# tejank10/AlphaGo.jl

Measured on AMD Instinct MI355X. Metric: self-play positions/sec (9x9, tower=10, 400 readouts), higher is better.
Workload: dtype f32

## Files before the change

alphago.jl_amd/csrc/agz_nn.h:

```cpp
#pragma once
#include <algorithm>
#include <cstdint>
#include <functional>
#include <memory>
#include <vector>

#include "agz_common.h"

namespace agz {

constexpr int kC = 256;
constexpr int kCinStem = 17;
constexpr int kCinStemPad = 32;

struct ConvHost {
  int k = 3, cin = 0, cout = 0;
  std::vector<float> w, b, beta, gamma, mean, var;
  float eps = 1e-5f;
};
struct DenseHost {
  int in = 0, out = 0;
  std::vector<float> w, b;
};

// ... 57 lines not shown
  uint64_t param_version() const { return param_version_; }

  double flops_per_eval() const;
  double conv_flops_per_launch(int B) const { return 2.0 * B * P_ * 9.0 * kC * kC; }

 private:
  void pack();
  void stem(TowerForm form, const float* d_x32, const int* d_count, int bcap);
  void direct_tower(const int* d_count, int bcap);
  void f16_tower(const int* d_count, int bcap);
  void wino_tower(TowerForm form, const int* d_count, int bcap);
  void persistent_tower(const int* d_count, int bcap);
  struct LayerIO { const float *vin, *res; float *y, *vout; };
  LayerIO layer_io(int l, bool dense) const;
  void wino_layer(TowerForm form, int l, const LayerIO& io, const int* d_count, int bcap, hipStream_t st, int part = 0,
                  int parts = 1);
  template <class Layer> void run_chains(int chains, const Layer& layer);
  template <class Launch> void timed(int layers, const Launch& launch);

  int N_, P_, A_, tower_;
  hipStream_t stream_;
  ConvHost stem_, vconv_, pconv_;
  std::vector<ConvHost> tconv_;
  DenseHost vfc1_, vfc2_, pfc_;
  struct FluxSlot { int layer, kind; size_t off, n; };
  std::vector<FluxSlot> slots_;
  size_t flux_n_ = 0;
  DevBuf<float> d_flux_;
  bool derived_dirty_ = true;
  mutable bool host_stale_ = false;
  uint64_t param_version_ = 0;
  void upload_slot(const FluxSlot& s);
  void upload_host_all();
  const float* host_slot(const FluxSlot& s) const;

  DevBuf<float> d_wstem_, d_wtower_;
  DevBuf<float> d_scale_, d_shift_;
  DevBuf<float> d_head_;
  const float *d_vfc1w_ = nullptr, *d_vfc1b_ = nullptr, *d_vfc2w_ = nullptr, *d_vfc2b_ = nullptr, *d_pfcw_ = nullptr,
              *d_pfcb_ = nullptr;
  int bcap_ = 0;
  DevBuf<float> d_a_, d_b_, d_t_, d_vh_, d_ph_;
  int winograd_ = 1;
  DevBuf<float> d_uwino5_;
  bool packed5_ = false;
  DevBuf<float> d_uwino4_;
  bool packed4_ = false;
  static constexpr int kMaxTowerStreams = 4;
  int tower_streams_ = 2;
  hipStream_t streamx_[kMaxTowerStreams - 1] = {nullptr, nullptr, nullptr};
  hipEvent_t ev_fork_ = nullptr, ev_join_[kMaxTowerStreams - 1] = {nullptr, nullptr, nullptr};
  DevBuf<float> d_uwino_s_, d_scale_s_;
  bool packed_split_ = false;
  DevBuf<float> d_uwino_, d_vimg_, d_vimg2_;
  DevBuf<float> d_ustem_, d_ustem_s_;
  int precision_ = 0;
  bool packed16_ = false;
// ... 53 lines not shown
inline void wino_block_range(int blocks, int part, int parts, bool pairs, int& tb0, int& tb1) {
  AGZ_REQUIRE(parts >= 1 && part >= 0 && part < parts, AGZ_BAD_ARGUMENT, "tile-block range %d of %d", part, parts);
  int per = (blocks + parts - 1) / parts;
  if (pairs) per = (per + 1) & ~1;
  tb0 = std::min(blocks, part * per);
  tb1 = part + 1 == parts ? blocks : std::min(blocks, tb0 + per);
}
inline void wino_check_32bit(long blocks, int rows, int bcap, int N) {
  AGZ_REQUIRE((blocks + 1) * rows < (1L << 31) && (long)bcap * N * N * kC * 4 < (1L << 32), AGZ_BAD_ARGUMENT,
              "batch of %d positions at %dx%d: tile index / activation byte offset exceeds 32 bits", bcap, N, N);
}
void launch_wino_in(const float* x, float* vimg, const int* d_count, int bcap, int N, bool split, hipStream_t s,
                    int ns = kWinoStages, bool fixup = false);
void launch_wino_gemm(const float* vimg, const float* uimg, const float* scale, const float* shift, const float* res,
                      float* y, float* vnext, const int* d_count, int bcap, int N, int relu, bool split, hipStream_t s,
                      int ns = kWinoStages, int part = 0, int parts = 1);
bool wino_fusable(int N);
struct WinoTowerLayer {
  const float *v, *u, *scale, *shift, *res;
  float *y, *vnext;
  int mode, relu;
};
size_t wino_tower_sched_ints(int layers, int bcap, int N);
bool wino_tower_supported(hipStream_t s);
void launch_wino_tower(const void* d_layers, int layers, int* d_sched, const int* d_count, int bcap, int N, bool split, hipStream_t s);
constexpr int kWinoTowerErrWord = 8;
void wino_pack_weights_split(const ConvHost& c, float* out, int ns = kWinoStages);
float wino_split_descale();

void wino5_pack_weights(const ConvHost& c, float* out);
void launch_wino5_pack(const float* d_w, long wstride, int layers, float* d_out, hipStream_t s);
size_t wino5_weight_floats();
void launch_wino5_gemm(const float* vimg, const float* uimg, const float* scale, const float* shift, const float* res,
                       float* y, float* vnext, const int* d_count, int bcap, int N, int relu, hipStream_t s, int part = 0,
                       int parts = 1);

// ... 29 lines not shown
```

alphago.jl_amd/csrc/agz_nn.hip:

```cpp
#include "agz_nn.h"

#include <cmath>
#include <algorithm>
#include <cstring>

#include "../../include/agz_draws.h"

namespace agz {

typedef float f32x16 __attribute__((ext_vector_type(16)));


constexpr int BM = 128, BN = 128, BK = 32;
constexpr int LDS_STRIDE = BK + 4;

template <int CIN, bool TAPSPLIT = false>
__global__ __launch_bounds__(256, 2) void k_conv3x3_mfma(
    const float* __restrict__ x, const float* __restrict__ wt, const float* __restrict__ scale,
    const float* __restrict__ shift, const float* __restrict__ res, float* __restrict__ y,
    const int* __restrict__ d_count, int N, int relu, long ystride = 0) {
  constexpr int NCHUNK = 9 * CIN / BK;
  constexpr int CPT = CIN / BK;
  const int c_begin = TAPSPLIT ? (int)blockIdx.y * CPT : 0, c_end = TAPSPLIT ? c_begin + CPT : NCHUNK;
  if (TAPSPLIT) y += (long)blockIdx.y * ystride;
// ... 143 lines not shown
  const int lane = threadIdx.x & 63, wave = threadIdx.x >> 6;
#pragma unroll
  for (int o = 32; o > 0; o >>= 1) {
    const float t = __shfl_xor(v, o, 64);
    v = is_max ? fmaxf(v, t) : v + t;
  }
  __syncthreads();
  if (lane == 0) red[wave] = v;
  __syncthreads();
  float r = red[0];
#pragma unroll
  for (int w = 1; w < 4; ++w) r = is_max ? fmaxf(r, red[w]) : r + red[w];
  return r;
}

__global__ __launch_bounds__(256) void k_head_fc(
    const float* __restrict__ vh, const float* __restrict__ ph, const float* __restrict__ w1,
    const float* __restrict__ b1, const float* __restrict__ w2, const float* __restrict__ b2,
    const float* __restrict__ wp, const float* __restrict__ bp, float* __restrict__ pi,
    float* __restrict__ v, const int* __restrict__ d_count, int P, int A) {
  extern __shared__ __attribute__((aligned(16))) float sm[];
  float* vin = sm;
  float* pin = sm + P;
  float* logit = pin + 2 * P;
  float* red = logit + A;
  const int b = blockIdx.x;
  if (b >= *d_count) return;
  const int tid = threadIdx.x;
  for (int i = tid; i < P; i += 256) {
    vin[i] = vh[(long)b * P + i];
    pin[i] = ph[((long)b * P + i) * 2 + 0];
    pin[P + i] = ph[((long)b * P + i) * 2 + 1];
  }
  __syncthreads();
  float lmax = -INFINITY;
  for (int o = tid; o < A; o += 256) {
    float z = bp[o];
    for (int i = 0; i < 2 * P; ++i) z += wp[o + (long)A * i] * pin[i];
    logit[o] = z;
    lmax = fmaxf(lmax, z);
  }
  const float mx = block_reduce(lmax, true, red);
  float lsum = 0.f;
  for (int o = tid; o < A; o += 256) {
    const float e = expf(logit[o] - mx);
    logit[o] = e;
    lsum += e;
  }
  const float sum = block_reduce(lsum, false, red);
  for (int o = tid; o < A; o += 256) pi[(long)b * A + o] = logit[o] / sum;
  float h = b1[tid];
  for (int i = 0; i < P; ++i) h += w1[tid + 256 * i] * vin[i];
  h = fmaxf(h, 0.f);
  const float s = block_reduce(h * w2[tid], false, red);
  if (tid == 0) v[b] = tanhf(s + b2[0]);
}


__global__ __launch_bounds__(128) void k_feats_from_deltas(
    const int8_t* __restrict__ boards, const int8_t* __restrict__ deltas, const int32_t* __restrict__ ndeltas,
    const int8_t* __restrict__ to_play, int B, int N, float* __restrict__ x32, float* __restrict__ whcn) {
  const int b = blockIdx.x;
  if (b >= B) return;
  const int P = N * N;
  const int nd = ndeltas[b];
  const int tp = to_play[b];
  for (int p = threadIdx.x; p < P; p += blockDim.x) {
    int cur = boards[(long)b * P + p];
    float f[32];
#pragma unroll
// ... 447 lines not shown

void Net::reserve(int bcap) {
  if (precision_ == 1 && tower_ > 0 && d_ha_.n < ((size_t)std::max(bcap, bcap_) * P_ + 256) * kC) {
    const size_t n = ((size_t)std::max(bcap, bcap_) * P_ + 256) * kC;
    d_ha_.alloc(n);
    d_hb_.alloc(n);
    d_ht_.alloc(n);
  }
  if (bcap <= bcap_) return;
  const size_t rows = (size_t)bcap * P_;
  d_a_.alloc(rows * kC);
  d_b_.alloc(rows * kC);
  d_t_.alloc(rows * kC);
  d_vh_.alloc(rows);
  d_ph_.alloc(rows * 2);
  if (tower_ > 0) {
    const size_t vf = std::max(wino_v_floats(bcap, (N_ + 2) / 3), wino4_applies(N_) ? wino4_v_floats(bcap, N_) : (size_t)0);
    d_vimg_.alloc(vf);
    d_vimg2_.alloc(vf);
  }
  bcap_ = bcap;
}

static inline int conv_grid(int bcap, int P) { return ceil_div((long)bcap * P, BM) * (kC / BN); }
int conv3x3_direct_blocks(int bcap, int N) { return conv_grid(bcap, N * N); }

void launch_conv3x3_direct(const float* x, const float* wt, const float* scale, const float* shift, const float* res,
                           float* y, const int* d_count, int bcap, int N, int relu, int cin_pad, hipStream_t s) {
  const int grid = conv_grid(bcap, N * N);
  if (cin_pad == kCinStemPad)
// ... 143 lines not shown
    timed(1, [&] {
      launch_conv16_dma(d_ht_.p, d_wi16_.p + iper * l2, sc + (size_t)l2 * kC, sh + (size_t)l2 * kC,
                        first ? (const void*)a : (const void*)cur, first ? 1 : 0, last ? (void*)d_b_.p : (void*)nxt,
                        last ? 1 : 0, d_count, bcap, N_, 1, stream_);
    });
    std::swap(cur, nxt);
  }
}

Net::LayerIO Net::layer_io(int l, bool dense) const {
  if (l % 2 == 0) return {d_vimg_.p, nullptr, dense ? d_t_.p : nullptr, d_vimg2_.p};
  const bool odd = (l / 2) % 2;
  return {d_vimg2_.p, odd ? d_b_.p : d_a_.p, odd ? d_a_.p : d_b_.p, l + 1 == 2 * tower_ ? nullptr : d_vimg_.p};
}

void Net::wino_layer(TowerForm form, int l, const LayerIO& io, const int* d_count, int bcap, hipStream_t st, int part, int parts) {
  const float* sc = d_scale_.p + (size_t)(l + 1) * kC;
  const float* sh = d_shift_.p + (size_t)(l + 1) * kC;
  if (form == TowerForm::Wino4) {
    launch_wino4_gemm(io.vin, d_uwino4_.p + wino4_weight_floats() * l, sc, sh, io.res, io.y, io.vout, d_count, bcap, N_, 1, st,
                      part, parts, io.y && !io.res && wino4_paired(N_));
    if (io.vout && !wino4_whole_boards(N_)) launch_wino4_in(io.y, io.vout, d_count, bcap, N_, st, true, part, parts);
  } else if (form == TowerForm::Wino5) {
    launch_wino5_gemm(io.vin, d_uwino5_.p + wino5_weight_floats() * l, sc, sh, io.res, io.y, io.vout, d_count, bcap, N_, 1, st,
                      part, parts);
  } else {
    const bool split = precision_ == 2;
    const float* u = (split ? d_uwino_s_.p : d_uwino_.p) + wino_weight_floats() * l;
    launch_wino_gemm(io.vin, u, split ? d_scale_s_.p + (size_t)l * kC : sc, sh, io.res, io.y, io.vout, d_count, bcap, N_, 1, split,
                     st, kWinoStages, part, parts);
    if (io.vout && !wino_fusable(N_)) launch_wino_in(io.y, io.vout, d_count, bcap, N_, split, st, kWinoStages, true);
  }
}

void Net::wino_tower(TowerForm form, const int* d_count, int bcap) {
  const bool f44 = form == TowerForm::Wino4;
  const bool dense = f44 ? !wino4_whole_boards(N_) : !wino_fusable(N_);
  const int T = f44 ? (N_ + 3) / 4 : (N_ + 2) / 3;
  const int chains = dense && !f44 ? 1 : chain_count(tower_streams_, (long)bcap * T * T, f44 ? 64 : 63);
  run_chains(chains, [&](int l, int part, hipStream_t st) {
    wino_layer(form, l, layer_io(l, dense), d_count, bcap, st, part, chains);
  });
}

void Net::persistent_tower(const int* d_count, int bcap) {
  const bool split = precision_ == 2;
  const float* usrc = split ? d_uwino_s_.p : d_uwino_.p;
  const float* sc = split ? d_scale_s_.p : d_scale_.p + kC;
  const float* sh = d_shift_.p + kC;
  const int nl = 2 * tower_;
  std::vector<WinoTowerLayer> tab(nl);
  for (int l = 0; l < nl; ++l) {
    const LayerIO io = layer_io(l, false);
    tab[l] = {io.vin, usrc + wino_weight_floats() * l, sc + (size_t)l * kC, sh + (size_t)l * kC, io.res, io.y, io.vout,
              (io.y ? 1 : 0) | (io.vout ? 2 : 0), 1};
  }
  const size_t tbytes = sizeof(WinoTowerLayer) * tab.size();
  if (tower_layers_host_.size() != tbytes || std::memcmp(tower_layers_host_.data(), tab.data(), tbytes) != 0) {
    AGZ_HIP(hipStreamSynchronize(stream_));
    tower_layers_host_.assign((const char*)tab.data(), (const char*)tab.data() + tbytes);
    d_tower_layers_.ensure(tbytes);
    AGZ_HIP(hipMemcpy(d_tower_layers_.p, tower_layers_host_.data(), tbytes, hipMemcpyHostToDevice));
  }
  d_tower_sched_.ensure(wino_tower_sched_ints(nl, bcap, N_));
  if (!tower_err_) {
    AGZ_HIP(hipHostMalloc((void**)&tower_err_, sizeof(int32_t), hipHostMallocDefault));
    *tower_err_ = 0;
  }
  timed(nl, [&] { launch_wino_tower(d_tower_layers_.p, nl, d_tower_sched_.p, d_count, bcap, N_, split, stream_); });
  (void)hipMemcpyAsync(tower_err_, d_tower_sched_.p + kWinoTowerErrWord, sizeof(int32_t), hipMemcpyDeviceToHost, stream_);
// ... 3 lines not shown
  check_async_error();
  TowerForm form = tower_form();
  if (form == TowerForm::Wino4) wino4_validate(bcap, N_);
  pack();
  reserve(bcap);
  if (prof_on_ && prof_fwd_ < kProfMax)
    (void)hipMemcpyAsync(&prof_counts_[prof_fwd_], d_count, sizeof(int32_t), hipMemcpyDeviceToHost, stream_);
  stem(form, d_x32, d_count, bcap);
  if (form == TowerForm::Wino3Persistent && !wino_tower_supported(stream_)) form = TowerForm::Wino3;
  switch (form) {
    case TowerForm::Direct: direct_tower(d_count, bcap); break;
    case TowerForm::F16: f16_tower(d_count, bcap); break;
    case TowerForm::Wino3Persistent: persistent_tower(d_count, bcap); break;
    default: wino_tower(form, d_count, bcap); break;
  }
  const float* x = form == TowerForm::F16 || tower_ % 2 ? d_b_.p : d_a_.p;
  const int hgrid = std::min(ceil_div((long)bcap * P_, 4), 256 * 16);
  hipLaunchKernelGGL(k_head_conv, dim3(hgrid), dim3(256), 0, stream_, x, d_head_.p, d_vh_.p, d_ph_.p, d_count, P_);
  const size_t smem = sizeof(float) * (size_t)(3 * P_ + A_ + 4);
  hipLaunchKernelGGL(k_head_fc, dim3(bcap), dim3(256), smem, stream_, (const float*)d_vh_.p,
                     (const float*)d_ph_.p, d_vfc1w_, d_vfc1b_, d_vfc2w_, d_vfc2b_, d_pfcw_,
                     d_pfcb_, d_pi, d_v, d_count, P_, A_);
  if (prof_on_ && prof_fwd_ < kProfMax) prof_fwd_++;
  AGZ_HIP(hipGetLastError());
}

__global__ __launch_bounds__(256) void k_mfma_f32_sustained(int iters, float* out) {
  typedef float f32x16 __attribute__((ext_vector_type(16)));
  f32x16 acc[8];
#pragma unroll
  for (int i = 0; i < 8; ++i)
#pragma unroll
    for (int e = 0; e < 16; ++e) acc[i][e] = 0.f;
  const float a = 1.f + threadIdx.x * 1e-6f, b = 0.5f;
  for (int it = 0; it < iters; ++it) {
#pragma unroll
    for (int i = 0; i < 8; ++i) acc[i] = __builtin_amdgcn_mfma_f32_32x32x2f32(a, b, acc[i], 0, 0, 0);
// ... 143 lines not shown
```

alphago.jl_amd/csrc/agz_wino.hip:

```cpp
#include "agz_nn.h"
#include "agz_glds.h"

#include <algorithm>
#include <cmath>
#include <cstdio>
#include <cstdlib>
#include <cstring>
#include <type_traits>

namespace agz {

typedef float f32x16 __attribute__((ext_vector_type(16)));

constexpr int WT = 64;
constexpr int WC = 64;
constexpr int WK = 4;
constexpr int WNS = kC / WK;
static_assert(WNS == kWinoStages && kCinStemPad == kWinoStemStages * WK, "stage counts of agz_nn.h");
constexpr int WXI = 25;
constexpr int WPL = 13;
constexpr int A_STAGE = WPL * WT * 8;
constexpr int B_STAGE = WPL * WC * 8;
constexpr int STAGE = A_STAGE + B_STAGE;

__host__ __device__ __forceinline__ int wino_v_off(int xi, int row, int h) {
  return (xi >> 1) * (WT * 8) + (xi & 1) * (WT * 4) + row * 4 + 2 * ((h + (row >> 4)) & 1);
}

typedef _Float16 h8 __attribute__((ext_vector_type(8)));
typedef _Float16 h4 __attribute__((ext_vector_type(4)));
constexpr float kSplitV = 8.f, kSplitU = 1024.f;
__host__ __device__ __forceinline__ void split_half(float x, _Float16& hi, _Float16& lo) {
  hi = (_Float16)x;
  lo = (_Float16)(x - (float)hi);
// ... 11 lines not shown
  const int lo = (ti > 0 ? T : 0) + (tj > 0 ? 1 : 0), hi = (ti < T - 1 ? T : 0) + (tj < T - 1 ? 1 : 0);
  return row - lo >= 0 && row + hi < WT;
}


__device__ __forceinline__ void bt5(float x0, float x1, float x2, float x3, float x4, float* r) {
  r[3] = x3 - x1;
  r[0] = __builtin_fmaf(2.f, x0 - x2, r[3]);
  r[4] = __builtin_fmaf(-2.f, r[3], x4 - x2);
  r[1] = __builtin_fmaf(2.f, x1, x2 - x3);
  r[2] = __builtin_fmaf(-2.f, x1, __builtin_fmaf(3.f, x2, -x3));
}

template <int TPB, bool NT, bool SPLIT = false, int NS = WNS, bool FIXUP = false>
__global__ __launch_bounds__(256) void k_wino_in(const float* __restrict__ x, float* __restrict__ vimg,
                                                  const int* __restrict__ d_count, int N, int T) {
  static_assert(TPB == 32, "the copy-out below moves 32-row chunks");
  constexpr int LPT = 256 / TPB;
  constexpr int SP = LPT / 2;
  constexpr int CH = TPB * 4;
  constexpr int IMG = 26 * CH + 8;
  __shared__ __attribute__((aligned(16))) float img[SP * IMG];
  const int P = N * N, TT = T * T;
  const int RPB = wino_rows_per_block(T);
  const long Mt = (long)(*d_count) * TT;
  constexpr int PARTS = WT / TPB;
  const int tb = blockIdx.x / PARTS, part = blockIdx.x % PARTS;
  if ((long)tb * RPB + part * TPB >= Mt) return;
  const int hs = threadIdx.x % LPT, h = hs & 1, sl = hs >> 1;
  const int tl = threadIdx.x / LPT;
  const int row = part * TPB + tl;
// ... 11 lines not shown
      const bool ok = live && pi >= 0 && pi < N && pj >= 0 && pj < N;
      off[u * 5 + v] = ok ? (b * P + pi + N * pj) * (NS * WK) : -1;
    }
  float* mine = img + sl * IMG + tl * 4 + (SPLIT ? 0 : 2 * ((h + (row >> 4)) & 1));
  if (SPLIT) { mine[25 * CH + h] = 0.f; mine[25 * CH + 2 + h] = 0.f; }
  else *reinterpret_cast<float2*>(mine + 25 * CH) = make_float2(0.f, 0.f);
  float* gdst = vimg + (long)tb * NS * A_STAGE + part * CH;
  const int cq = threadIdx.x / TPB, cl = threadIdx.x % TPB;
  bool copy_row = true;
  if (FIXUP) {
    const int crow = part * TPB + cl;
    const long ctile = (long)tb * RPB + crow;
    const int ct = (int)(ctile % TT);
    copy_row = !(crow < RPB && ctile < Mt && wino_tile_fused(T, crow, ct / T, ct % T));
  }
  for (int sg = 0; sg < NS / SP; ++sg) {
    const int st = sg * SP + sl;
    float2 d[25];
#pragma unroll
    for (int q = 0; q < 25; ++q)
      d[q] = off[q] >= 0 ? *reinterpret_cast<const float2*>(x + off[q] + st * WK + 2 * h) : make_float2(0.f, 0.f);
    float tx[25], ty[25];
#pragma unroll
    for (int v = 0; v < 5; ++v) {
      float r[5];
      bt5(d[0 * 5 + v].x, d[1 * 5 + v].x, d[2 * 5 + v].x, d[3 * 5 + v].x, d[4 * 5 + v].x, r);
#pragma unroll
      for (int i = 0; i < 5; ++i) tx[i * 5 + v] = r[i];
      bt5(d[0 * 5 + v].y, d[1 * 5 + v].y, d[2 * 5 + v].y, d[3 * 5 + v].y, d[4 * 5 + v].y, r);
#pragma unroll
      for (int i = 0; i < 5; ++i) ty[i * 5 + v] = r[i];
    }
    if (sg) __syncthreads();
#pragma unroll
    for (int i = 0; i < 5; ++i) {
      float rx[5], ry[5];
// ... 9 lines not shown
          *reinterpret_cast<h2*>(mine + (i * 5 + j) * CH + h) = (h2){xh, yh};
          *reinterpret_cast<h2*>(mine + (i * 5 + j) * CH + 2 + h) = (h2){xl, yl};
        } else {
          *reinterpret_cast<float2*>(mine + (i * 5 + j) * CH) = make_float2(rx[j], ry[j]);
        }
      }
    }
    __syncthreads();
#pragma unroll
    for (int r = 0; r < 13; ++r) {
      const int c = r * 8 + cq, s4 = c / 26, xi = c % 26;
      typedef float f32x4 __attribute__((ext_vector_type(4)));
      const f32x4 v = *reinterpret_cast<const f32x4*>(img + s4 * IMG + xi * CH + cl * 4);
      f32x4* gp = reinterpret_cast<f32x4*>(gdst + (long)(sg * SP + s4) * A_STAGE + (xi >> 1) * (WT * 8) + (xi & 1) * (WT * 4) + cl * 4);
      if (FIXUP && !copy_row) continue;
      if (NT) __builtin_nontemporal_store(v, gp);
      else *gp = v;
    }
  }
}

constexpr int IMG_FLOATS = WT * 9 * WC;

template <bool SPLIT, int NS, bool COH>
__device__ __forceinline__ void wino_wg(
    float* __restrict__ lds, int* __restrict__ ptab, const float* __restrict__ vimg, const float* __restrict__ uimg,
    const float* __restrict__ scale, const float* __restrict__ shift, const float* __restrict__ res, float* __restrict__ y,
    float* __restrict__ vnext, const long Mt, const int N, const int T, const int relu, const int tb, const int cb, const int MODE,
    const int tid) {
  const int P = N * N, TT = T * T;
  const int RPB = wino_rows_per_block(T);
  const int lane = tid & 63;
  const int wave = __builtin_amdgcn_readfirstlane(tid >> 6);
  const int wm = wave & 1, wn = wave >> 1;
  const int l31 = lane & 31, hi = lane >> 5;
  const float* asrc = vimg + (long)tb * NS * A_STAGE;
  const float* bsrc = uimg + (long)cb * NS * B_STAGE;
  const unsigned lds0 = (unsigned)(size_t)(__attribute__((address_space(3))) float*)&lds[0];

  auto dma = [&](int st, int buf, int j) {
    const int c = 13 * wave + j;
    if (j == 12 && (wave & 1)) return;
    const float* g = wave < 2 ? asrc + (long)st * A_STAGE + c * 256 : bsrc + (long)st * B_STAGE + (c - 26) * 256;
    if constexpr (COH) glds16s_l2(g, (unsigned)lane * 16u, lds0 + (unsigned)(buf * STAGE + c * 256) * 4u);
// ... 110 lines not shown
      if (t < WXI) load(L, t, ra[t % RING], rb[t % RING]);
      else if (next) load(Ln, t - WXI, ra[t % RING], rb[t % RING]);
      constexpr int D0 = SPLIT ? 0 : 6;
      if (more && k >= D0 && k < D0 + PW) {
        __builtin_amdgcn_sched_barrier(0);
        dma(st + 2, dbuf, k - D0);
        __builtin_amdgcn_sched_barrier(0);
      }
      if (first) mma0(k, ra[k % RING], rb[k % RING]);
      else mma(k, ra[k % RING], rb[k % RING]);
    }
    buf = nbuf;
  };
  static_assert(NS >= 4, "stage 0 is peeled off the loop");
  stage(0, std::true_type{}, std::true_type{}, std::true_type{});
  for (int st = 1; st < NS - 2; ++st) stage(st, std::true_type{}, std::true_type{}, std::false_type{});
  stage(NS - 2, std::false_type{}, std::true_type{}, std::false_type{});
  stage(NS - 1, std::false_type{}, std::false_type{}, std::false_type{});

  static_assert(WXI == 25, "the pad below lists the accumulators of transform columns 3 and 4");
  asm volatile("s_nop 15\n\ts_nop 15"
               : "+v"(acc[3]), "+v"(acc[4]), "+v"(acc[8]), "+v"(acc[9]), "+v"(acc[13]), "+v"(acc[14]), "+v"(acc[18]),
                 "+v"(acc[19]), "+v"(acc[23]), "+v"(acc[24]));

  __syncthreads();
  float* img = lds;
  static_assert(IMG_FLOATS + WC <= 3 * STAGE, "tile image (+ the block of zeros phase 2 reads for off-board points) exceeds the stage buffers");
  if (tid < WC) img[IMG_FLOATS + tid] = 0.f;
  const bool pass1b = (MODE & 1) != 0;
  if (res) {
    static_assert(WT * 9 / 4 == 4 * 36, "36 residual pieces per wave");
#pragma unroll
    for (int n = 0; n < 36; ++n) rdma(n);
  }
  {
    const int col = wn * 32 + l31;
    const float sc = scale[cb * WC + col], sh = shift[cb * WC + col];
    const float relu_lo = relu ? 0.f : -3.0e38f;
    f32x16 o[9];
    {
      f32x16 tmp[3][5];
#pragma unroll
      for (int jj = 0; jj < 5; ++jj) {
        const int j = (jj + 3) % 5;
// ... 32 lines not shown
            rr[ee][k] = decltype(with_res)::value ? *((lds_f*)(size_t)pa[ee][k >> 2] + (k & 3) * (WT * WC)) : 0.f;
        }
#pragma unroll
        for (int ee = 0; ee < 4; ++ee)
#pragma unroll
          for (int k = 0; k < 9; ++k) {
            float v = o[k][e0 + ee] * sc + sh + rr[ee][k];
            v = fmaxf(v, relu_lo);
            *((lds_f*)(size_t)pa[ee][k >> 2] + (k & 3) * (WT * WC)) = v;
          }
      }
    };
    if (res) rows(std::true_type{});
    else rows(std::false_type{});
  }
  __syncthreads();
  typedef float f32x4 __attribute__((ext_vector_type(4)));
  if (pass1b) {
    constexpr int PER = WT * 9 * (WC / 4) / 256;
    const int cg4 = 4 * ((tid ^ (tid >> 4)) & 15);
    f32x4* ip0 = reinterpret_cast<f32x4*>(img) + tid;
    const int* pt0 = ptab + (tid >> 4);
    int offs[PER];
#pragma unroll
    for (int i = 0; i < PER; ++i) offs[i] = pt0[16 * i];
#pragma unroll
    for (int i0 = 0; i0 < PER; i0 += 12) {
      f32x4 v[12];
#pragma unroll
      for (int j = 0; j < 12; ++j) v[j] = ip0[256 * (i0 + j)];
#pragma unroll
      for (int j = 0; j < 12; ++j)
        if ((MODE & 1) && offs[i0 + j] >= 0) *reinterpret_cast<f32x4*>(y + offs[i0 + j] + cg4) = v[j];
// ... 83 lines not shown
          v4 = __builtin_bit_cast(f32x4, pk);
        } else {
          v4 = (f32x4){p0[0], p0[1], p1[0], p1[1]};
        }
        f32x4* gp = reinterpret_cast<f32x4*>(g + (xi >> 1) * (WT * 8) + (xi & 1) * (WT * 4));
        if (emit) __builtin_nontemporal_store(v4, gp);
      }
    }
  }
}

template <int MODE, bool SPLIT = false, int NS = WNS>
__global__ __launch_bounds__(256, 1) void k_wino_gemm4(
    const float* __restrict__ vimg, const float* __restrict__ uimg, const float* __restrict__ scale,
    const float* __restrict__ shift, const float* __restrict__ res, float* __restrict__ y,
    float* __restrict__ vnext, const int* __restrict__ d_count, int N, int T, int relu, int tb0, int tb1) {
  __shared__ __attribute__((aligned(256))) float lds[3 * STAGE];
  __shared__ int ptab[WT * 9];
  const long Mt = (long)(*d_count) * (T * T);
  const int bid = blockIdx.x;
  const int xcd = bid & 7, jb = bid >> 3;
  const int cb = jb & 3;
  const int tb = tb0 + xcd + 8 * (jb >> 2);
  if (tb >= tb1 || (long)tb * wino_rows_per_block(T) >= Mt) return;
  wino_wg<SPLIT, NS, false>(lds, ptab, vimg, uimg, scale, shift, res, y, vnext, Mt, N, T, relu, tb, cb, MODE, (int)threadIdx.x);
}

typedef WinoTowerLayer TowerLayer;
static_assert(kWinoTowerErrWord == 8, "");
constexpr int kTowerErr = kWinoTowerErrWord, kTowerDone = 64;
constexpr int kTowerSpinLimit = 1 << 22;

template <bool SPLIT>
__global__ __launch_bounds__(256, 1) void k_wino_tower(const TowerLayer* __restrict__ layers, int nl, int* __restrict__ sched,
                                                       int blocks_cap, const int* __restrict__ d_count, int N, int T, int order) {
  __shared__ __attribute__((aligned(256))) float lds[3 * STAGE];
  __shared__ int ptab[WT * 9];
  __shared__ int s_bc;
  const int tid = threadIdx.x;
  unsigned xcc;
// ... 31 lines not shown
      int spins = 0;
      while (__hip_atomic_load(flag, __ATOMIC_RELAXED, __HIP_MEMORY_SCOPE_AGENT) < 4) {
        __builtin_amdgcn_s_sleep(8);
        if (++spins > kTowerSpinLimit || ((spins & 1023) == 0 && __hip_atomic_load(&sched[kTowerErr], __ATOMIC_RELAXED, __HIP_MEMORY_SCOPE_AGENT))) {
          atomicOr(&sched[kTowerErr], 2);
          s_bc = 1;
          break;
        }
      }
    }
    __syncthreads();
    if (s_bc) return;
    const TowerLayer L = layers[l];
    int t = tid;
    asm volatile("" : "+v"(t));
    wino_wg<SPLIT, WNS, true>(lds, ptab, L.v, L.u, L.scale, L.shift, L.res, L.y, L.vnext, Mt, N, T, L.relu, tb, cb, L.mode, t);
    asm volatile("s_waitcnt vmcnt(0)" ::: "memory");
    __syncthreads();
    if (tid == 0) {
      int* flag = done + (size_t)l * blocks_cap + tb;
      if (__hip_atomic_fetch_add(flag, 1, __ATOMIC_RELAXED, __HIP_MEMORY_SCOPE_AGENT) != 3) {
        int spins = 0;
        while (__hip_atomic_load(flag, __ATOMIC_RELAXED, __HIP_MEMORY_SCOPE_AGENT) < 4 && ++spins < kTowerSpinLimit) __builtin_amdgcn_s_sleep(2);
      }
    }
  }
}

__global__ void k_xcd_census(int* out) {
  __shared__ float hog[150 * 1024 / 4];
  unsigned xcc;
// ... 67 lines not shown

size_t wino_weight_floats(int ns) { return (size_t)(kC / WC) * ns * B_STAGE; }
long wino_blocks(int bcap, int T) {
  const long rpb = wino_rows_per_block(T);
  return ((long)bcap * T * T + rpb - 1) / rpb;
}
size_t wino_v_floats(int bcap, int T) { return (size_t)wino_blocks(bcap, T) * WNS * A_STAGE; }
bool wino_fusable(int N) { return wino_whole_boards((N + 2) / 3); }

void launch_wino_in(const float* x, float* vimg, const int* d_count, int bcap, int N, bool split, hipStream_t s, int ns,
                    bool fixup) {
  const int T = (N + 2) / 3;
  const int blocks = (int)wino_blocks(bcap, T);
  AGZ_REQUIRE(!fixup || (ns == kWinoStages && !wino_whole_boards(T)), AGZ_BAD_ARGUMENT, "fix-up transform: dense tile blocks, tower layers");
#define WIN_LAUNCH(SPLIT_, NS_, FIXUP_) \
  hipLaunchKernelGGL((k_wino_in<32, true, SPLIT_, NS_, FIXUP_>), dim3(2 * blocks), dim3(256), 0, s, x, vimg, d_count, N, T)
  constexpr int S = kWinoStemStages;
  switch ((fixup ? 4 : ns == S ? 2 : 0) | (split ? 1 : 0)) {
    case 5: WIN_LAUNCH(true, WNS, true); break;
    case 4: WIN_LAUNCH(false, WNS, true); break;
    case 3: WIN_LAUNCH(true, S, false); break;
    case 2: WIN_LAUNCH(false, S, false); break;
    case 1: WIN_LAUNCH(true, WNS, false); break;
    default: WIN_LAUNCH(false, WNS, false); break;
  }
#undef WIN_LAUNCH
}

void launch_wino_gemm(const float* vimg, const float* uimg, const float* scale, const float* shift, const float* res,
                      float* y, float* vnext, const int* d_count, int bcap, int N, int relu, bool split, hipStream_t s, int ns, int part,
                      int parts) {
  const int T = (N + 2) / 3;
  const int all_blocks = (int)wino_blocks(bcap, T);
  int tb0, tb1;
  wino_block_range(all_blocks, part, parts, false, tb0, tb1);
  AGZ_REQUIRE(parts == 1 || wino_whole_boards(T), AGZ_BAD_ARGUMENT, "F(3x3,3x3): %d layer chains need whole-board tile blocks", parts);
  if (tb1 <= tb0) return;
  const int blocks = tb1 - tb0;
  const int per_xcd = 4 * ((blocks + 7) / 8);
  const dim3 grid(8 * per_xcd), block(256);
  wino_check_32bit(all_blocks, WT, bcap, N);
  const bool stem = ns == kWinoStemStages;
  const int mode = vnext ? (y || stem ? 3 : 2) : 1;
#define WG_LAUNCH(MODE_, SPLIT_, NS_)                                                                                     \
  hipLaunchKernelGGL((k_wino_gemm4<MODE_, SPLIT_, NS_>), grid, block, 0, s, vimg, uimg, scale, shift, res, y, vnext, d_count, \
                     N, T, relu, tb0, tb1)
  constexpr int S = kWinoStemStages;
  switch (mode | (split ? 4 : 0) | (stem ? 8 : 0)) {
    case 15: WG_LAUNCH(3, true, S); break;
    case 13: WG_LAUNCH(1, true, S); break;
    case 11: WG_LAUNCH(3, false, S); break;
    case 9: WG_LAUNCH(1, false, S); break;
    case 7: WG_LAUNCH(3, true, WNS); break;
    case 6: WG_LAUNCH(2, true, WNS); break;
    case 5: WG_LAUNCH(1, true, WNS); break;
    case 3: WG_LAUNCH(3, false, WNS); break;
    case 2: WG_LAUNCH(2, false, WNS); break;
    default: WG_LAUNCH(1, false, WNS); break;
  }
#undef WG_LAUNCH
}
// ... 44 lines not shown
```

Before: 447.1.

## Fuse head 1x1 convs into last Winograd layer epilogue and trim stem stages

The last tower layer's Winograd GEMM epilogue now computes per-channel-block partial dot products for the value and policy 1x1 head convolutions, instead of writing the full activation. A new head FC kernel sums the four partials and applies BN/ReLU, which removes the separate head-conv launch and the full-activation write and read. The stem Winograd transform and GEMM also now process only the stages that cover the real 17 input channels rather than the padded 32. This adds a partial-sum buffer and epilogue complexity, and the fused path only applies when boards split into whole tile blocks.

```diff
diff --git a/alphago.jl_amd/csrc/agz_nn.h b/alphago.jl_amd/csrc/agz_nn.h
--- a/alphago.jl_amd/csrc/agz_nn.h
+++ b/alphago.jl_amd/csrc/agz_nn.h
@@ -95,7 +95,10 @@
   struct LayerIO { const float *vin, *res; float *y, *vout; };
   LayerIO layer_io(int l, bool dense) const;
   void wino_layer(TowerForm form, int l, const LayerIO& io, const int* d_count, int bcap, hipStream_t st, int part = 0,
-                  int parts = 1);
+                  int parts = 1, bool heads = false);
+  bool heads_fused(TowerForm form) const {
+    return (form == TowerForm::Wino3 || form == TowerForm::Wino3Persistent) && tower_ >= 1 && wino_fusable(N_);
+  }
   template <class Layer> void run_chains(int chains, const Layer& layer);
   template <class Launch> void timed(int layers, const Launch& launch);
 
@@ -122,6 +125,7 @@
               *d_pfcb_ = nullptr;
   int bcap_ = 0;
   DevBuf<float> d_a_, d_b_, d_t_, d_vh_, d_ph_;
+  DevBuf<float> d_hpart_;
   int winograd_ = 1;
   DevBuf<float> d_uwino5_;
   bool packed5_ = false;
@@ -205,12 +209,16 @@
                     int ns = kWinoStages, bool fixup = false);
 void launch_wino_gemm(const float* vimg, const float* uimg, const float* scale, const float* shift, const float* res,
                       float* y, float* vnext, const int* d_count, int bcap, int N, int relu, bool split, hipStream_t s,
-                      int ns = kWinoStages, int part = 0, int parts = 1);
+                      int ns = kWinoStages, int part = 0, int parts = 1, const float* hp = nullptr, float* hpart = nullptr,
+                      int hstride = 0);
 bool wino_fusable(int N);
 struct WinoTowerLayer {
   const float *v, *u, *scale, *shift, *res;
   float *y, *vnext;
   int mode, relu;
+  const float* hp;
+  float* hpart;
+  int hstride;
 };
 size_t wino_tower_sched_ints(int layers, int bcap, int N);
 bool wino_tower_supported(hipStream_t s);
diff --git a/alphago.jl_amd/csrc/agz_nn.hip b/alphago.jl_amd/csrc/agz_nn.hip
--- a/alphago.jl_amd/csrc/agz_nn.hip
+++ b/alphago.jl_amd/csrc/agz_nn.hip
@@ -181,6 +181,38 @@
   return r;
 }
 
+__device__ __forceinline__ void head_fc_tail(
+    float* sm, int b, const float* __restrict__ w1, const float* __restrict__ b1, const float* __restrict__ w2,
+    const float* __restrict__ b2, const float* __restrict__ wp, const float* __restrict__ bp, float* __restrict__ pi,
+    float* __restrict__ v, int P, int A) {
+  float* vin = sm;
+  float* pin = sm + P;
+  float* logit = pin + 2 * P;
+  float* red = logit + A;
+  const int tid = threadIdx.x;
+  float lmax = -INFINITY;
+  for (int o = tid; o < A; o += 256) {
+    float z = bp[o];
+    for (int i = 0; i < 2 * P; ++i) z += wp[o + (long)A * i] * pin[i];
+    logit[o] = z;
+    lmax = fmaxf(lmax, z);
+  }
+  const float mx = block_reduce(lmax, true, red);
+  float lsum = 0.f;
+  for (int o = tid; o < A; o += 256) {
+    const float e = expf(logit[o] - mx);
+    logit[o] = e;
+    lsum += e;
+  }
+  const float sum = block_reduce(lsum, false, red);
+  for (int o = tid; o < A; o += 256) pi[(long)b * A + o] = logit[o] / sum;
+  float h = b1[tid];
+  for (int i = 0; i < P; ++i) h += w1[tid + 256 * i] * vin[i];
+  h = fmaxf(h, 0.f);
+  const float s = block_reduce(h * w2[tid], false, red);
+  if (tid == 0) v[b] = tanhf(s + b2[0]);
+}
+
 __global__ __launch_bounds__(256) void k_head_fc(
     const float* __restrict__ vh, const float* __restrict__ ph, const float* __restrict__ w1,
     const float* __restrict__ b1, const float* __restrict__ w2, const float* __restrict__ b2,
@@ -189,38 +221,40 @@
   extern __shared__ __attribute__((aligned(16))) float sm[];
   float* vin = sm;
   float* pin = sm + P;
-  float* logit = pin + 2 * P;
-  float* red = logit + A;
   const int b = blockIdx.x;
   if (b >= *d_count) return;
-  const int tid = threadIdx.x;
-  for (int i = tid; i < P; i += 256) {
+  for (int i = threadIdx.x; i < P; i += 256) {
     vin[i] = vh[(long)b * P + i];
     pin[i] = ph[((long)b * P + i) * 2 + 0];
     pin[P + i] = ph[((long)b * P + i) * 2 + 1];
   }
   __syncthreads();
-  float lmax = -INFINITY;
-  for (int o = tid; o < A; o += 256) {
-    float z = bp[o];
-    for (int i = 0; i < 2 * P; ++i) z += wp[o + (long)A * i] * pin[i];
-    logit[o] = z;
-    lmax = fmaxf(lmax, z);
-  }
-  const float mx = block_reduce(lmax, true, red);
-  float lsum = 0.f;
-  for (int o = tid; o < A; o += 256) {
-    const float e = expf(logit[o] - mx);
-    logit[o] = e;
-    lsum += e;
-  }
-  const float sum = block_reduce(lsum, false, red);
-  for (int o = tid; o < A; o += 256) pi[(long)b * A + o] = logit[o] / sum;
-  float h = b1[tid];
-  for (int i = 0; i < P; ++i) h += w1[tid + 256 * i] * vin[i];
-  h = fmaxf(h, 0.f);
-  const float s = block_reduce(h * w2[tid], false, red);
-  if (tid == 0) v[b] = tanhf(s + b2[0]);
+  head_fc_tail(sm, b, w1, b1, w2, b2, wp, bp, pi, v, P, A);
+}
+
+__global__ __launch_bounds__(256) void k_head_fc_parts(
+    const float* __restrict__ hpart, int hstride, const float* __restrict__ hp, const float* __restrict__ w1,
+    const float* __restrict__ b1, const float* __restrict__ w2, const float* __restrict__ b2,
+    const float* __restrict__ wp, const float* __restrict__ bp, float* __restrict__ pi,
+    float* __restrict__ v, const int* __restrict__ d_count, int P, int A) {
+  extern __shared__ __attribute__((aligned(16))) float sm[];
+  float* vin = sm;
+  float* pin = sm + P;
+  const int b = blockIdx.x;
+  if (b >= *d_count) return;
+  const float sv = hp[768], tv = hp[769], s0 = hp[770], t0 = hp[771], s1 = hp[772], t1 = hp[773];
+  for (int i = threadIdx.x; i < P; i += 256) {
+    const float* q = hpart + ((long)b * P + i) * 3;
+    const long cs = (long)hstride * 3;
+    const float dv = ((q[0] + q[cs + 0]) + q[2 * cs + 0]) + q[3 * cs + 0];
+    const float d0 = ((q[1] + q[cs + 1]) + q[2 * cs + 1]) + q[3 * cs + 1];
+    const float d1 = ((q[2] + q[cs + 2]) + q[2 * cs + 2]) + q[3 * cs + 2];
+    vin[i] = fmaxf(dv * sv + tv, 0.f);
+    pin[i] = fmaxf(d0 * s0 + t0, 0.f);
+    pin[P + i] = fmaxf(d1 * s1 + t1, 0.f);
+  }
+  __syncthreads();
+  head_fc_tail(sm, b, w1, b1, w2, b2, wp, bp, pi, v, P, A);
 }
 
 
@@ -698,6 +732,7 @@
   d_t_.alloc(rows * kC);
   d_vh_.alloc(rows);
   d_ph_.alloc(rows * 2);
+  if (tower_ > 0 && wino_fusable(N_)) d_hpart_.alloc(rows * 3 * (kC / 64));
   if (tower_ > 0) {
     const size_t vf = std::max(wino_v_floats(bcap, (N_ + 2) / 3), wino4_applies(N_) ? wino4_v_floats(bcap, N_) : (size_t)0);
     d_vimg_.alloc(vf);
@@ -871,7 +906,8 @@
   return {d_vimg2_.p, odd ? d_b_.p : d_a_.p, odd ? d_a_.p : d_b_.p, l + 1 == 2 * tower_ ? nullptr : d_vimg_.p};
 }
 
-void Net::wino_layer(TowerForm form, int l, const LayerIO& io, const int* d_count, int bcap, hipStream_t st, int part, int parts) {
+void Net::wino_layer(TowerForm form, int l, const LayerIO& io, const int* d_count, int bcap, hipStream_t st, int part, int parts,
+                     bool heads) {
   const float* sc = d_scale_.p + (size_t)(l + 1) * kC;
   const float* sh = d_shift_.p + (size_t)(l + 1) * kC;
   if (form == TowerForm::Wino4) {
@@ -884,8 +920,9 @@
   } else {
     const bool split = precision_ == 2;
     const float* u = (split ? d_uwino_s_.p : d_uwino_.p) + wino_weight_floats() * l;
-    launch_wino_gemm(io.vin, u, split ? d_scale_s_.p + (size_t)l * kC : sc, sh, io.res, io.y, io.vout, d_count, bcap, N_, 1, split,
-                     st, kWinoStages, part, parts);
+    launch_wino_gemm(io.vin, u, split ? d_scale_s_.p + (size_t)l * kC : sc, sh, io.res, heads ? nullptr : io.y, io.vout, d_count,
+                     bcap, N_, 1, split, st, kWinoStages, part, parts, heads ? d_head_.p : nullptr, heads ? d_hpart_.p : nullptr,
+                     heads ? bcap_ * P_ : 0);
     if (io.vout && !wino_fusable(N_)) launch_wino_in(io.y, io.vout, d_count, bcap, N_, split, st, kWinoStages, true);
   }
 }
@@ -895,8 +932,9 @@
   const bool dense = f44 ? !wino4_whole_boards(N_) : !wino_fusable(N_);
   const int T = f44 ? (N_ + 3) / 4 : (N_ + 2) / 3;
   const int chains = dense && !f44 ? 1 : chain_count(tower_streams_, (long)bcap * T * T, f44 ? 64 : 63);
+  const bool fused = heads_fused(form);
   run_chains(chains, [&](int l, int part, hipStream_t st) {
-    wino_layer(form, l, layer_io(l, dense), d_count, bcap, st, part, chains);
+    wino_layer(form, l, layer_io(l, dense), d_count, bcap, st, part, chains, fused && l + 1 == 2 * tower_);
   });
 }
 
@@ -910,7 +948,13 @@
   for (int l = 0; l < nl; ++l) {
     const LayerIO io = layer_io(l, false);
     tab[l] = {io.vin, usrc + wino_weight_floats() * l, sc + (size_t)l * kC, sh + (size_t)l * kC, io.res, io.y, io.vout,
-              (io.y ? 1 : 0) | (io.vout ? 2 : 0), 1};
+              (io.y ? 1 : 0) | (io.vout ? 2 : 0), 1, nullptr, nullptr, 0};
+    if (l + 1 == nl) {
+      tab[l].y = nullptr;
+      tab[l].hp = d_head_.p;
+      tab[l].hpart = d_hpart_.p;
+      tab[l].hstride = bcap_ * P_;
+    }
   }
   const size_t tbytes = sizeof(WinoTowerLayer) * tab.size();
   if (tower_layers_host_.size() != tbytes || std::memcmp(tower_layers_host_.data(), tab.data(), tbytes) != 0) {
@@ -944,13 +988,19 @@
     case TowerForm::Wino3Persistent: persistent_tower(d_count, bcap); break;
     default: wino_tower(form, d_count, bcap); break;
   }
-  const float* x = form == TowerForm::F16 || tower_ % 2 ? d_b_.p : d_a_.p;
-  const int hgrid = std::min(ceil_div((long)bcap * P_, 4), 256 * 16);
-  hipLaunchKernelGGL(k_head_conv, dim3(hgrid), dim3(256), 0, stream_, x, d_head_.p, d_vh_.p, d_ph_.p, d_count, P_);
   const size_t smem = sizeof(float) * (size_t)(3 * P_ + A_ + 4);
-  hipLaunchKernelGGL(k_head_fc, dim3(bcap), dim3(256), smem, stream_, (const float*)d_vh_.p,
-                     (const float*)d_ph_.p, d_vfc1w_, d_vfc1b_, d_vfc2w_, d_vfc2b_, d_pfcw_,
-                     d_pfcb_, d_pi, d_v, d_count, P_, A_);
+  if (heads_fused(form)) {
+    hipLaunchKernelGGL(k_head_fc_parts, dim3(bcap), dim3(256), smem, stream_, (const float*)d_hpart_.p, bcap_ * P_,
+                       (const float*)d_head_.p, d_vfc1w_, d_vfc1b_, d_vfc2w_, d_vfc2b_, d_pfcw_, d_pfcb_, d_pi, d_v, d_count, P_,
+                       A_);
+  } else {
+    const float* x = form == TowerForm::F16 || tower_ % 2 ? d_b_.p : d_a_.p;
+    const int hgrid = std::min(ceil_div((long)bcap * P_, 4), 256 * 16);
+    hipLaunchKernelGGL(k_head_conv, dim3(hgrid), dim3(256), 0, stream_, x, d_head_.p, d_vh_.p, d_ph_.p, d_count, P_);
+    hipLaunchKernelGGL(k_head_fc, dim3(bcap), dim3(256), smem, stream_, (const float*)d_vh_.p,
+                       (const float*)d_ph_.p, d_vfc1w_, d_vfc1b_, d_vfc2w_, d_vfc2b_, d_pfcw_,
+                       d_pfcb_, d_pi, d_v, d_count, P_, A_);
+  }
   if (prof_on_ && prof_fwd_ < kProfMax) prof_fwd_++;
   AGZ_HIP(hipGetLastError());
 }
diff --git a/alphago.jl_amd/csrc/agz_wino.hip b/alphago.jl_amd/csrc/agz_wino.hip
--- a/alphago.jl_amd/csrc/agz_wino.hip
+++ b/alphago.jl_amd/csrc/agz_wino.hip
@@ -18,6 +18,8 @@
 constexpr int WNS = kC / WK;
 static_assert(WNS == kWinoStages && kCinStemPad == kWinoStemStages * WK, "stage counts of agz_nn.h");
 constexpr int WXI = 25;
+constexpr int kStemRun = (kCinStem + WK - 1) / WK;
+static_assert(kStemRun >= 4 && kStemRun <= kWinoStemStages, "the K loop peels one stage in front and two behind");
 constexpr int WPL = 13;
 constexpr int A_STAGE = WPL * WT * 8;
 constexpr int B_STAGE = WPL * WC * 8;
@@ -59,7 +61,7 @@
 
 template <int TPB, bool NT, bool SPLIT = false, int NS = WNS, bool FIXUP = false>
 __global__ __launch_bounds__(256) void k_wino_in(const float* __restrict__ x, float* __restrict__ vimg,
-                                                  const int* __restrict__ d_count, int N, int T) {
+                                                  const int* __restrict__ d_count, int N, int T, int ns_run) {
   static_assert(TPB == 32, "the copy-out below moves 32-row chunks");
   constexpr int LPT = 256 / TPB;
   constexpr int SP = LPT / 2;
@@ -101,12 +103,13 @@
     const int ct = (int)(ctile % TT);
     copy_row = !(crow < RPB && ctile < Mt && wino_tile_fused(T, crow, ct / T, ct % T));
   }
-  for (int sg = 0; sg < NS / SP; ++sg) {
+  const int nrun = NS == kWinoStemStages ? ns_run : NS;
+  for (int sg = 0; sg < (nrun + SP - 1) / SP; ++sg) {
     const int st = sg * SP + sl;
     float2 d[25];
 #pragma unroll
     for (int q = 0; q < 25; ++q)
-      d[q] = off[q] >= 0 ? *reinterpret_cast<const float2*>(x + off[q] + st * WK + 2 * h) : make_float2(0.f, 0.f);
+      d[q] = off[q] >= 0 && st < nrun ? *reinterpret_cast<const float2*>(x + off[q] + st * WK + 2 * h) : make_float2(0.f, 0.f);
     float tx[25], ty[25];
 #pragma unroll
     for (int v = 0; v < 5; ++v) {
@@ -146,6 +149,7 @@
       const f32x4 v = *reinterpret_cast<const f32x4*>(img + s4 * IMG + xi * CH + cl * 4);
       f32x4* gp = reinterpret_cast<f32x4*>(gdst + (long)(sg * SP + s4) * A_STAGE + (xi >> 1) * (WT * 8) + (xi & 1) * (WT * 4) + cl * 4);
       if (FIXUP && !copy_row) continue;
+      if (NS == kWinoStemStages && sg * SP + s4 >= nrun) continue;
       if (NT) __builtin_nontemporal_store(v, gp);
       else *gp = v;
     }
@@ -159,7 +163,7 @@
     float* __restrict__ lds, int* __restrict__ ptab, const float* __restrict__ vimg, const float* __restrict__ uimg,
     const float* __restrict__ scale, const float* __restrict__ shift, const float* __restrict__ res, float* __restrict__ y,
     float* __restrict__ vnext, const long Mt, const int N, const int T, const int relu, const int tb, const int cb, const int MODE,
-    const int tid) {
+    const int tid, const int ns_run, const float* __restrict__ hp, float* __restrict__ hpart, const int hstride) {
   const int P = N * N, TT = T * T;
   const int RPB = wino_rows_per_block(T);
   const int lane = tid & 63;
@@ -300,9 +304,15 @@
   };
   static_assert(NS >= 4, "stage 0 is peeled off the loop");
   stage(0, std::true_type{}, std::true_type{}, std::true_type{});
-  for (int st = 1; st < NS - 2; ++st) stage(st, std::true_type{}, std::true_type{}, std::false_type{});
-  stage(NS - 2, std::false_type{}, std::true_type{}, std::false_type{});
-  stage(NS - 1, std::false_type{}, std::false_type{}, std::false_type{});
+  if constexpr (NS == kWinoStemStages) {
+    for (int st = 1; st < ns_run - 2; ++st) stage(st, std::true_type{}, std::true_type{}, std::false_type{});
+    stage(ns_run - 2, std::false_type{}, std::true_type{}, std::false_type{});
+    stage(ns_run - 1, std::false_type{}, std::false_type{}, std::false_type{});
+  } else {
+    for (int st = 1; st < NS - 2; ++st) stage(st, std::true_type{}, std::true_type{}, std::false_type{});
+    stage(NS - 2, std::false_type{}, std::true_type{}, std::false_type{});
+    stage(NS - 1, std::false_type{}, std::false_type{}, std::false_type{});
+  }
 
   static_assert(WXI == 25, "the pad below lists the accumulators of transform columns 3 and 4");
   asm volatile("s_nop 15\n\ts_nop 15"
@@ -314,6 +324,11 @@
   static_assert(IMG_FLOATS + WC <= 3 * STAGE, "tile image (+ the block of zeros phase 2 reads for off-board points) exceeds the stage buffers");
   if (tid < WC) img[IMG_FLOATS + tid] = 0.f;
   const bool pass1b = (MODE & 1) != 0;
+  const bool heads = MODE == 1 && hpart != nullptr;
+  constexpr int HW = IMG_FLOATS + WC;
+  static_assert(HW + 3 * WC <= 3 * STAGE, "head weights behind the tile image exceed the stage buffers");
+  float hwv = 0.f;
+  if (heads && tid < 3 * WC) hwv = hp[(tid >> 6) * kC + cb * WC + (tid & 63)];
   if (res) {
     static_assert(WT * 9 / 4 == 4 * 36, "36 residual pieces per wave");
 #pragma unroll
@@ -376,9 +391,35 @@
     if (res) rows(std::true_type{});
     else rows(std::false_type{});
   }
+  if (heads && tid < 3 * WC) img[HW + tid] = hwv;
   __syncthreads();
   typedef float f32x4 __attribute__((ext_vector_type(4)));
-  if (pass1b) {
+  if (heads) {
+    const f32x4* hw4 = reinterpret_cast<const f32x4*>(img + HW);
+    for (int k = wave; k < 9; k += 4) {
+      const int X = k * WT + lane;
+      const int off = ptab[X];
+      const f32x4* px = reinterpret_cast<const f32x4*>(img + X * WC);
+      float s0 = 0.f, s1 = 0.f, s2 = 0.f;
+#pragma unroll
+      for (int g = 0; g < WC / 4; ++g) {
+        const f32x4 v = px[g ^ (lane & 15)];
+        const f32x4 a = hw4[g], b = hw4[WC / 4 + g], c = hw4[2 * (WC / 4) + g];
+#pragma unroll
+        for (int e = 0; e < 4; ++e) {
+          s0 = g + e == 0 ? v[e] * a[e] : __builtin_fmaf(v[e], a[e], s0);
+          s1 = g + e == 0 ? v[e] * b[e] : __builtin_fmaf(v[e], b[e], s1);
+          s2 = g + e == 0 ? v[e] * c[e] : __builtin_fmaf(v[e], c[e], s2);
+        }
+      }
+      if (off >= 0) {
+        float* o = hpart + ((size_t)cb * (size_t)hstride + (size_t)((unsigned)off / (unsigned)kC)) * 3;
+        o[0] = s0;
+        o[1] = s1;
+        o[2] = s2;
+      }
+    }
+  } else if (pass1b) {
     constexpr int PER = WT * 9 * (WC / 4) / 256;
     const int cg4 = 4 * ((tid ^ (tid >> 4)) & 15);
     f32x4* ip0 = reinterpret_cast<f32x4*>(img) + tid;
@@ -492,7 +533,8 @@
 __global__ __launch_bounds__(256, 1) void k_wino_gemm4(
     const float* __restrict__ vimg, const float* __restrict__ uimg, const float* __restrict__ scale,
     const float* __restrict__ shift, const float* __restrict__ res, float* __restrict__ y,
-    float* __restrict__ vnext, const int* __restrict__ d_count, int N, int T, int relu, int tb0, int tb1) {
+    float* __restrict__ vnext, const int* __restrict__ d_count, int N, int T, int relu, int tb0, int tb1, int ns_run,
+    const float* __restrict__ hp, float* __restrict__ hpart, int hstride) {
   __shared__ __attribute__((aligned(256))) float lds[3 * STAGE];
   __shared__ int ptab[WT * 9];
   const long Mt = (long)(*d_count) * (T * T);
@@ -501,7 +543,7 @@
   const int cb = jb & 3;
   const int tb = tb0 + xcd + 8 * (jb >> 2);
   if (tb >= tb1 || (long)tb * wino_rows_per_block(T) >= Mt) return;
-  wino_wg<SPLIT, NS, false>(lds, ptab, vimg, uimg, scale, shift, res, y, vnext, Mt, N, T, relu, tb, cb, MODE, (int)threadIdx.x);
+  wino_wg<SPLIT, NS, false>(lds, ptab, vimg, uimg, scale, shift, res, y, vnext, Mt, N, T, relu, tb, cb, MODE, (int)threadIdx.x, ns_run, hp, hpart, hstride);
 }
 
 typedef WinoTowerLayer TowerLayer;
@@ -563,7 +605,7 @@
     const TowerLayer L = layers[l];
     int t = tid;
     asm volatile("" : "+v"(t));
-    wino_wg<SPLIT, WNS, true>(lds, ptab, L.v, L.u, L.scale, L.shift, L.res, L.y, L.vnext, Mt, N, T, L.relu, tb, cb, L.mode, t);
+    wino_wg<SPLIT, WNS, true>(lds, ptab, L.v, L.u, L.scale, L.shift, L.res, L.y, L.vnext, Mt, N, T, L.relu, tb, cb, L.mode, t, WNS, L.hp, L.hpart, L.hstride);
     asm volatile("s_waitcnt vmcnt(0)" ::: "memory");
     __syncthreads();
     if (tid == 0) {
@@ -661,7 +703,7 @@
   const int blocks = (int)wino_blocks(bcap, T);
   AGZ_REQUIRE(!fixup || (ns == kWinoStages && !wino_whole_boards(T)), AGZ_BAD_ARGUMENT, "fix-up transform: dense tile blocks, tower layers");
 #define WIN_LAUNCH(SPLIT_, NS_, FIXUP_) \
-  hipLaunchKernelGGL((k_wino_in<32, true, SPLIT_, NS_, FIXUP_>), dim3(2 * blocks), dim3(256), 0, s, x, vimg, d_count, N, T)
+  hipLaunchKernelGGL((k_wino_in<32, true, SPLIT_, NS_, FIXUP_>), dim3(2 * blocks), dim3(256), 0, s, x, vimg, d_count, N, T, ns == kWinoStemStages ? kStemRun : ns)
   constexpr int S = kWinoStemStages;
   switch ((fixup ? 4 : ns == S ? 2 : 0) | (split ? 1 : 0)) {
     case 5: WIN_LAUNCH(true, WNS, true); break;
@@ -676,7 +718,7 @@
 
 void launch_wino_gemm(const float* vimg, const float* uimg, const float* scale, const float* shift, const float* res,
                       float* y, float* vnext, const int* d_count, int bcap, int N, int relu, bool split, hipStream_t s, int ns, int part,
-                      int parts) {
+                      int parts, const float* hp, float* hpart, int hstride) {
   const int T = (N + 2) / 3;
   const int all_blocks = (int)wino_blocks(bcap, T);
   int tb0, tb1;
@@ -689,9 +731,11 @@
   wino_check_32bit(all_blocks, WT, bcap, N);
   const bool stem = ns == kWinoStemStages;
   const int mode = vnext ? (y || stem ? 3 : 2) : 1;
+  AGZ_REQUIRE(!hpart || (hp && !y && !vnext && !stem && wino_whole_boards(T) && hstride >= bcap * N * N), AGZ_BAD_ARGUMENT,
+              "heads in the epilogue: the tower's last layer (no y, no next V), whole-board tile blocks");
 #define WG_LAUNCH(MODE_, SPLIT_, NS_)                                                                                     \
   hipLaunchKernelGGL((k_wino_gemm4<MODE_, SPLIT_, NS_>), grid, block, 0, s, vimg, uimg, scale, shift, res, y, vnext, d_count, \
-                     N, T, relu, tb0, tb1)
+                     N, T, relu, tb0, tb1, stem ? kStemRun : ns, hp, hpart, hstride)
   constexpr int S = kWinoStemStages;
   switch (mode | (split ? 4 : 0) | (stem ? 8 : 0)) {
     case 15: WG_LAUNCH(3, true, S); break;
```

Result: no change. 449.2 (median of 6 runs) (+0.5%).
